# AvishaiBarnoy/membrane_solver

Measured on AMD Instinct MI355X. Metric: minimizer steps/sec (energy+grad+CG) on 2M-facet icosphere, higher is better.
Workload: dtype f64

## Files before the change

include/membrane_hip.h:

```cpp
#ifndef MEMBRANE_HIP_H
#define MEMBRANE_HIP_H

#include <stddef.h>
#include <stdint.h>

#ifdef __cplusplus
extern "C" {
#endif

#define MS_OK 0
#define MS_ERR_INVALID (-1)
#define MS_ERR_HIP (-2)
#define MS_ERR_TILE_CAPACITY (-3)
#define MS_ERR_STATE (-4)
#define MS_ERR_NOMEM (-5)

#define MS_MOD_SURFACE 1u
#define MS_MOD_BENDING 2u
#define MS_MOD_VOLUME_PENALTY 4u
#define MS_CON_VOLUME 8u
#define MS_TRACK_VOLUME 16u
#define MS_MOD_TILT 32u
#define MS_MOD_BENDING_TILT 64u
#define MS_MOD_TILT_SMOOTH 128u
// ... 266 lines not shown
int ms_rebind_state(ms_ctx *ctx, void *device_base, size_t bytes);

int ms_device_buffer(ms_ctx *ctx, int buffer, void **dev_ptr, size_t *bytes);
int ms_shard_info(ms_ctx *ctx, int64_t *nvp, int64_t *row0, int64_t *row1,
                  int64_t *rows_per_shard);
int ms_tile_stats(ms_ctx *ctx, int64_t *n_tiles, int64_t *facet_instances,
                  int64_t *max_halo, int64_t *lds_bytes_energy,
                  int64_t *lds_bytes_gradient);

#define MS_PROF_KINDS 13
int ms_profile_enable(ms_ctx *ctx, int on);
int ms_profile_read(ms_ctx *ctx, double total_ms[MS_PROF_KINDS],
                    int64_t launches[MS_PROF_KINDS]);

int ms_queue_stats(ms_ctx *ctx, int64_t stats[8]);
int ms_exec_stats(ms_ctx *ctx, int64_t stats[4]);
int ms_resident_stats(ms_ctx *ctx, int64_t stats[4]);

#define MS_PIN_STAGE_FIXED 0
#define MS_PIN_STAGE_PLANE_GROUP 1
#define MS_PIN_STAGE_CIRCLE_GROUP 2
#define MS_PIN_OP_PLANE 0
#define MS_PIN_OP_CIRCLE 1
#define MS_PIN_GRAD_PLANE 0
#define MS_PIN_GRAD_CIRCLE 1
#define MS_PIN_GRAD_RADIAL 2
#define MS_PIN_LANE_SKIP 0
#define MS_PIN_LANE_PROJECT 1
int ms_set_pins(ms_ctx *ctx, int n_params, const double *params, int n_stages, const int32_t *stage_kind,
                const int32_t *stage_param, const int32_t *stage_off, const int32_t *item_row,
// ... 36 lines not shown
```

membrane_solver_amd/_lib.py:

```python

from __future__ import annotations

import ctypes
import os
import subprocess

_PKG = os.path.dirname(os.path.abspath(__file__))
LIB_PATH = os.environ.get("MEMBRANE_HIP_LIB") or os.path.join(_PKG, "libmembrane_hip.so")
_CSRC = os.path.join(_PKG, "csrc")

MS_OK = 0
MS_ERR = {-1: "MS_ERR_INVALID", -2: "MS_ERR_HIP", -3: "MS_ERR_TILE_CAPACITY",
          -4: "MS_ERR_STATE", -5: "MS_ERR_NOMEM"}

MS_MOD_SURFACE = 1
MS_MOD_BENDING = 2
MS_MOD_VOLUME_PENALTY = 4
MS_CON_VOLUME = 8
MS_TRACK_VOLUME = 16
MS_MOD_TILT = 32
MS_MOD_BENDING_TILT = 64
MS_MOD_TILT_SMOOTH = 128
MS_MOD_TILT_IN, MS_MOD_TILT_OUT, MS_MOD_TILT_SMOOTH_IN, MS_MOD_TILT_SMOOTH_OUT = 256, 512, 1024, 2048
MS_MOD_BENDING_TILT_IN, MS_MOD_BENDING_TILT_OUT = 4096, 8192
# ... 158 lines not shown
    "ms_shard_exchange_count": (ctypes.c_int64, [_P]),
    "ms_shard_chain_stats": (ctypes.c_int, [_P, _I64]),
    "ms_shard_comm_ranks": (ctypes.c_int, [_P]),
    "ms_shard_peer_memory_kind": (ctypes.c_int, [_P]),
    "ms_state_bytes": (ctypes.c_size_t, [_P]),
    "ms_rebind_state": (ctypes.c_int, [_P, _P, ctypes.c_size_t]),
    "ms_fetch_scalars": (ctypes.c_int, [_P, _D]),
    "ms_store_scalars": (ctypes.c_int, [_P, _D]),
    "ms_device_buffer": (ctypes.c_int, [_P, ctypes.c_int, ctypes.POINTER(_P),
                                        ctypes.POINTER(ctypes.c_size_t)]),
    "ms_shard_info": (ctypes.c_int, [_P, _I64, _I64, _I64, _I64]),
    "ms_tile_stats": (ctypes.c_int, [_P, _I64, _I64, _I64, _I64, _I64]),
    "ms_profile_enable": (ctypes.c_int, [_P, ctypes.c_int]),
    "ms_profile_read": (ctypes.c_int, [_P, _D, _I64]),
    "ms_queue_stats": (ctypes.c_int, [_P, _I64]),
    "ms_exec_stats": (ctypes.c_int, [_P, _I64]),
    "ms_resident_stats": (ctypes.c_int, [_P, _I64]),
    "ms_set_pins": (ctypes.c_int, [_P, ctypes.c_int, _D, ctypes.c_int, _I32, _I32, _I32, _I32, _I32, ctypes.c_int,
                                   ctypes.c_int, _I32, _I32, _I32, ctypes.c_int, _I32, _I32, _I32]),
    "ms_enforce_pins": (ctypes.c_int, [_P]),
    "ms_pin_stats": (ctypes.c_int, [_P, _I64]),
    "ms_tsearch_stats": (ctypes.c_int, [_P, _I64]),
    "ms_exec_trace": (ctypes.c_int, [_P, ctypes.c_int, _D, ctypes.c_int, ctypes.POINTER(ctypes.c_int)]),
    "ms_shard_peer_export": (ctypes.c_int, [_P, _P]),
    "ms_shard_peer_open": (ctypes.c_int, [_P, _P]),
    "ms_shard_peer_local": (ctypes.c_int, [_P, ctypes.POINTER(_P), ctypes.POINTER(_P)]),
    "ms_shard_peer_set_pointers": (ctypes.c_int, [_P, ctypes.POINTER(_P), ctypes.POINTER(_P)]),
    "ms_shard_peer_set_barrier": (ctypes.c_int, [_P, _P, _P]),
    "ms_plan_tiling": (ctypes.c_int, [ctypes.c_int, ctypes.c_int, _D, _I32, ctypes.c_int, ctypes.c_int,
                                      _I64, _I32]),
# ... 88 lines not shown
```

membrane_solver_amd/csrc/ms_api_ctx.inc:

```
struct StageCtl {
  const uint32_t* cur_gate = nullptr;
  uint32_t cur_gate_want = 0;
  bool cur_gate_fold_only = false;
  bool cur_check_ran = false;
  uint32_t* cur_dec = nullptr;
  double cur_rhs[MS_MAX_TRIALS] = {0};
  const double* cur_rhs_dev = nullptr;
  uint32_t cur_extra_mask = 0;
  int cur_go_kind = 0;
  uint32_t* cur_go = nullptr;
  double cur_go_val[6] = {0};
  int cur_parity = 0;
  int pair_on = 0;
  bool pair_lean = false;
  double pair_alpha[MS_MAX_TRIALS] = {0};
  double* pair_scal2 = nullptr;
  bool multi_any_slot = false;
  bool defer_dir = false;
  bool energy_tilt_only = false;
  bool proj_at_x_in_normals = false;
};
struct CarryState {
  bool dir_implicit = false;
  bool pd_neg_pg = false;
  bool kc_pending = false;
  int kc_parity = 0;
  bool bt_valid = false;
  double* last_g = nullptr;
  bool cg_have_history = false;
  int cg_iter_count = 0;
  bool factors_valid = false;
  bool carry_valid = false;
  bool grad_valid = false;
  bool maxg2_valid = false;
};
struct ms_ctx {
  int device = 0;
  hipStream_t stream = nullptr;
// ... 70 lines not shown
    bool implicit = false;
    double alpha0 = 0, energy0 = 0, beta = 0, c1 = 0, tol2p = 0, lim = 0;
    RoundPlanT plan;
  } ahead;
  bool ahead_enable = true;
  int steps_left = 0;
  bool ahead_allowed = false;
  uint32_t dir_deferred_mask = 0;
  bool dir_pending[2] = {false, false};
  uint32_t dir_mask[2] = {0, 0};
  uint32_t* kc_gate[2] = {nullptr, nullptr};
  bool last_hist_descent = false;
  long q_ahead = 0, q_adopted = 0, q_dropped = 0;
  int kc_stepper = 0;
  bool kc_use_history = false;
  uint32_t* d_dec = nullptr;
  static constexpr int N_DEC = 16;
  unsigned long long* h_err = nullptr;
  unsigned long long* d_h_err = nullptr;
  long queue_mismatches = 0;
  long q_rounds = 0, q_multi = 0, q_wasted = 0, q_side_accepts = 0;
  int escalate_after = 3;
  bool pair_enable = true;
  bool escalate = true;
  int pair_force = 0;
  bool lbt_normals_current = false;
  bool tenergy_enable = true;
  bool tsearch_enable = true;
  bool tsearch_first_single = true;
  int64_t tsearch_launches = 0, tsearch_trials = 0;
// ... 158 lines not shown
```

membrane_solver_amd/csrc/ms_api_misc.inc:

```
size_t ms_state_bytes(const ms_ctx* c) {
  if (!c) return 0;
  return sizeof(double) * (8 * 3 * (size_t)c->til.nvp + 2 * (size_t)c->til.nvp);
}

int ms_rebind_state(ms_ctx* c, void* device_base, size_t bytes) {
  if (!c || !device_base) return fail(c, MS_ERR_INVALID, "ms_rebind_state: NULL argument");
  const size_t need = ms_state_bytes(c);
  if (bytes < need) return fail(c, MS_ERR_INVALID, "ms_rebind_state: buffer smaller than ms_state_bytes");
  HIPCHK(c, hipStreamSynchronize(S(c)));
  HIPCHK(c, hipMemcpy(device_base, c->state, need, hipMemcpyDeviceToDevice));
  double* nb = static_cast<double*>(device_base);
  for (int b = 0; b <= MS_BUF_FA; ++b) c->buf[b] = nb + (c->buf[b] - c->state);
  c->carry.last_g = nb + (c->carry.last_g - c->state);
  if (c->own_state) HIPCHK(c, hipFree(c->state));
  c->state = nb;
  c->own_state = false;
  return MS_OK;
}

int ms_fetch_scalars(ms_ctx* c, double* out) {
  if (!c || !out) return MS_ERR_INVALID;
  int rc = fetch(c);
  if (rc) return rc;
  memcpy(out, c->h_scal, sizeof(double) * MS_NSCAL);
// ... 48 lines not shown
                                                      (c->params.modules & MS_CON_VOLUME) != 0, !c->deterministic);
  return MS_OK;
}

int ms_queue_stats(ms_ctx* c, int64_t stats[8]) {
  if (!c || !stats) return MS_ERR_INVALID;
  for (int k = 0; k < 8; ++k) stats[k] = 0;
  stats[0] = c->q_rounds;
  stats[1] = c->q_multi;
  stats[2] = c->q_wasted;
  stats[3] = c->q_side_accepts;
  stats[4] = c->queue_mismatches;
  stats[5] = c->q_ahead;
  stats[6] = c->q_adopted;
  stats[7] = c->q_dropped;
  return MS_OK;
}

int ms_resident_stats(ms_ctx* c, int64_t stats[4]) {
  if (!c || !stats) return MS_ERR_INVALID;
  stats[0] = c->resident_ok;
  stats[1] = c->resident_launches;
  stats[2] = c->resident_steps;
  stats[3] = c->resident_bails;
  return MS_OK;
}

int ms_tsearch_stats(ms_ctx* c, int64_t stats[2]) {
  if (!c || !stats) return MS_ERR_INVALID;
  stats[0] = c->tsearch_launches;
// ... 320 lines not shown
```

membrane_solver_amd/csrc/ms_api_phases.inc:

```
namespace {

inline hipStream_t S(ms_ctx* c) {
  if (c->exec_on) (void)c->exec.flush();
  return c->stream;
}
int pin_grad_run(ms_ctx* c, bool volrow);
inline int exec_flush(ms_ctx* c) {
  if (!c->exec_on) return MS_OK;
  const hipError_t e = c->exec.flush();
  if (e == hipSuccess) return MS_OK;
  c->err = std::string("k_exec launch: ") + hipGetErrorString(e);
  return MS_ERR_HIP;
}

inline int zero_doubles(ms_ctx* c, double* p, size_t bytes) {
  if (c->exec_on) {
    ExecMemsetArgs a;
    a.p = p;
    a.n = (int64_t)(bytes / sizeof(double));
    const hipError_t e = c->exec.push(CK_MEMSET, 0, 0, 0, 1, 0, 0, &a, sizeof(a));
    if (e == hipSuccess) return MS_OK;
    c->err = std::string("k_exec record: ") + hipGetErrorString(e);
    return MS_ERR_HIP;
  }
// ... 672 lines not shown
    if (!used) return fail(c, MS_ERR_STATE, "tilt energy pass: planned but not launched");
  }
  if (reduce_now) {
    constexpr uint32_t core = (1u << MS_S_ESURF) | (1u << MS_S_VOL) | (1u << MS_S_EBEND) | (1u << MS_S_MINEDGE2) |
                              (1u << MS_S_GUARD);
    int rc = reduce_slots(c, tilt_only ? (energy_mask(modules) & ~core) : energy_mask(modules));
    if (rc) return rc;
  }
  if (bend && write_factors) c->carry.factors_valid = !use_dir;
  if (!lbt) c->factors_leaflet = 0;
  c->carry.bt_valid = (bt || lbt) && !use_dir;
  return MS_OK;
}

int phase_gradient(ms_ctx* c, uint32_t modules_in, double* g_out, bool accumulate, int dir_mode = 0,
                   bool reduce_now = true) {
  uint32_t modules = modules_in;
  if ((modules & (MS_MOD_BENDING | MS_MOD_BENDING_TILT | MS_LEAFLET_BT)) && !c->carry.factors_valid)
    return fail(c, MS_ERR_STATE, "gradient pass needs the bending factors of an energy pass at x");
  if (modules & MS_MOD_BENDING_TILT)
    modules = (modules & ~MS_MOD_BENDING_TILT) | MS_MOD_BENDING;
  int lbt_order[2] = {0, 0}, n_lbt = 0;
  if (modules & MS_LEAFLET_BT) {
    if (dir_mode) return fail(c, MS_ERR_STATE, "bending_tilt_in/out cannot use the fused direction pass");
    if (modules & MS_MOD_BENDING) return fail(c, MS_ERR_STATE, "bending together with bending_tilt_in/out is outside the device path");
    if (c->params.bending_grad_mode != MS_GRAD_ANALYTIC)
      return fail(c, MS_ERR_STATE, "bending_tilt_in/out: only bending_gradient_mode=analytic is on the device path");
    for (int l = 2; l >= 1; --l)
      if (modules & c->tf[l].mod_bt) lbt_order[n_lbt++] = l;
    if (n_lbt == 2 && c->factors_leaflet == lbt_order[1]) std::swap(lbt_order[0], lbt_order[1]);
    modules |= MS_MOD_BENDING;
// ... 5 lines not shown
  a.x = c->buf[MS_BUF_X];
  a.fK = c->buf[MS_BUF_FK];
  a.fA = c->buf[MS_BUF_FA];
  a.g = g_out;
  a.gC = (modules & MS_CON_VOLUME) ? c->buf[MS_BUF_GC] : nullptr;
  a.partials = c->d_partials;
  a.scal = c->d_scal;
  a.modules = modules;
  a.bending_grad_mode = c->params.bending_grad_mode;
  a.volume_stiffness = c->params.volume_stiffness;
  a.target_volume = c->params.target_volume;
  a.area_stiffness = c->area_stiffness;
  a.target_area = c->target_area;
  a.accumulate = accumulate ? 1 : 0;
  a.dir_mode = dir_mode;
  a.d = c->buf[MS_BUF_D];
  a.pg = c->buf[MS_BUF_PG];
  a.pd = c->buf[MS_BUF_PD];
  a.pd_neg_pg = (dir_mode == 2 && c->carry.pd_neg_pg) ? 1 : 0;
  a.gate = c->stage().cur_gate;
  a.gate_want = c->stage().cur_gate_want;
  a.atomic = c->deterministic ? 0 : 1;
  a.bt_vert = nullptr;
  a.tilts = nullptr;
  a.div_sign = 1.0;
  if (n_lbt == 0) {
    ProfScope ps(c, gradient_lean_instance(a) ? 9 : 1, a.gate, a.gate_want);
    HIPCHK(c, launch_gradient(a, c->cap, c->til.max_ent, c->stream));
  }
  for (int k = 0; k < n_lbt; ++k) {
    TiltField& f = c->tf[lbt_order[k]];
// ... 13 lines not shown
    if (k > 0) {
      al.modules = MS_MOD_BENDING;
      al.gC = nullptr;
      al.accumulate = 1;
    }
    {
      ProfScope ps(c, 1);
      HIPCHK(c, launch_gradient(al, c->cap, c->til.max_ent, c->stream));
    }
    int rc = bt_pass_f(c, f, 3, false, 0.0, f.tilts);
    if (rc) return rc;
  }
  if (dir_mode) {
    c->carry.last_g = g_out;
    c->carry.dir_implicit = false;
  }
  bool added_after = n_lbt > 0;
  for (int k = 0; k < 3 && g_out; ++k) {
    TiltField& f = c->tf[k];
    if (modules & f.mod_tilt) {
      int rc = tilt_pass_f(c, f, 1, false, 0.0);
      if (rc) return rc;
      added_after = true;
    }
    if (k > 0 && (modules & f.mod_dt)) {
      int rc = disk_target_pass(c, f, 1, false, 0.0, f.tilts, true, false);
      if (rc) return rc;
      added_after = true;
    }
  }
  if (added_after && g_out && (modules & MS_CON_VOLUME))
    HIPCHK(c, launch_row_dot(c->tile0, c->tile1, c->til.nv, c->til.own, g_out, c->buf[MS_BUF_GC], c->d_partials,
                             c->til.n_tiles, c->stream));
  if (reduce_now) return reduce_slots(c, dir_mode ? MASK_DIR : MASK_GRAD);
  return MS_OK;
}

int phase_direction(ms_ctx* c, int stepper, bool use_history, bool g_finalized = false) {
  const bool use_con = (c->params.modules & MS_CON_VOLUME) != 0 && c->pin_lane != MS_PIN_LANE_SKIP;
  const StageCtl& st = c->stage();
  c->carry.dir_implicit = false;
  {
  ProfScope ps(c, 2, st.cur_gate, st.cur_gate_want);
  HIPCHK(c, launch_direction(c->tile0, c->tile1, c->til.nv, c->til.own, c->d_vflags, c->buf[MS_BUF_G],
                             c->buf[MS_BUF_GC], c->buf[MS_BUF_D], c->buf[MS_BUF_PG],
                             c->buf[MS_BUF_PD], c->d_scal, use_con ? 1 : 0,
                             (stepper == MS_STEPPER_CG && use_history) ? 1 : 0, c->d_partials,
                             c->til.n_tiles, (g_finalized && !use_con) ? 0 : 1, c->stream, st.cur_gate,
                             st.cur_gate_want,
                             (stepper == MS_STEPPER_CG && use_history && c->carry.pd_neg_pg) ? 1 : 0,
                             (stepper == MS_STEPPER_CG && c->precond) ? 1 : 0));
  }
  c->carry.last_g = c->buf[MS_BUF_G];
  return reduce_slots(c, MASK_DIR);
}

void put_mailbox(ms_ctx* c, int sl, double v) {
  c->h_scal[sl] = v;
  unsigned long long bits;
  memcpy(&bits, &v, sizeof(double));
  __atomic_store_n(&c->h_seq[2 * sl], bits, __ATOMIC_RELAXED);
  __atomic_store_n(&c->h_seq[2 * sl + 1], bits ^ c->expected[sl], __ATOMIC_RELAXED);
}

const char* box_name(ms_ctx* c, const void* h_seq);
bool trace_queue();

int check_queue_error(ms_ctx* c) {
  if (!c->h_err) return MS_OK;
  const unsigned long long e = __atomic_load_n(c->h_err, __ATOMIC_ACQUIRE);
// ... 109 lines not shown
    if (c->params.modules & f.mod_bt) e[1] += c->h_scal[f.s_ebt];
    if (c->params.modules & f.mod_dt) e[3] += c->h_scal[f.s_edt];
  }
}

int queue_energy_and_gradient(ms_ctx* c, int stepper, bool use_history, bool skip_energy = false) {
  const uint32_t mods = c->params.modules;
  const bool constraint = (mods & (MS_CON_VOLUME | MS_TILT_SHAPE_MODS)) != 0 || (stepper == MS_STEPPER_CG && c->precond) ||
                          c->pin_lane == MS_PIN_LANE_PROJECT;
  const bool penalty = skip_energy || (mods & (MS_MOD_VOLUME_PENALTY | MS_MOD_AREA_PENALTY)) != 0;
  int rc = MS_OK;
  if (!skip_energy) rc = phase_energy(c, mods, false, 0.0, false, false, true, penalty);
  if (rc) return rc;
  if (!constraint) {
    const int dir_mode = (stepper == MS_STEPPER_CG && use_history) ? 2 : 1;
    rc = phase_gradient(c, mods, c->buf[MS_BUF_G], false, dir_mode, false);
    if (rc) return rc;
    return reduce_slots(c, (penalty ? 0u : energy_mask(mods)) | MASK_DIR);
  }
  rc = phase_gradient(c, mods, c->buf[MS_BUF_G], false, 0, false);
  if (rc) return rc;
  rc = pin_grad_run(c, (mods & MS_CON_VOLUME) != 0);
  if (rc) return rc;
  const uint32_t gmask = (mods & (MS_CON_VOLUME | MS_TILT_SHAPE_MODS)) ? MASK_GRAD : 0u;
  const uint32_t fmask = (penalty ? 0u : energy_mask(mods)) | gmask;
  if (fmask) rc = reduce_slots(c, fmask);
  if (rc) return rc;
  return phase_direction(c, stepper, use_history);
}

template <typename Tp>
// ... 45 lines not shown
```

membrane_solver_amd/csrc/ms_api_shard.inc:

```
int ms_phase_energy(ms_ctx* c, int use_direction, double alpha, int write_trial, int guard,
                    int write_bending_factors) {
  if (!c) return MS_ERR_INVALID;
  if ((c->params.modules & MS_ANY_TILT_MODS) && c->shard_count != 1)
    return fail(c, MS_ERR_STATE, "the tilt module is not sharded yet (single GPU only)");
  return phase_energy(c, c->params.modules, use_direction != 0, alpha, write_trial != 0, guard != 0,
                      write_bending_factors != 0);
}

int ms_phase_gradient(ms_ctx* c) {
  if (!c) return MS_ERR_INVALID;
  c->carry.grad_valid = false;
  return phase_gradient(c, c->params.modules, c->buf[MS_BUF_G], false);
}

int ms_phase_direction(ms_ctx* c, int stepper, int use_history) {
  if (!c) return MS_ERR_INVALID;
  c->precond = false;
  return phase_direction(c, stepper, use_history != 0);
}

int ms_phase_accept(ms_ctx* c, int keep_history) {
  if (!c) return MS_ERR_INVALID;
  std::swap(c->buf[MS_BUF_X], c->buf[MS_BUF_XT]);
  c->carry.factors_valid = false;
  c->carry.carry_valid = c->carry.grad_valid = c->carry.bt_valid = c->carry.maxg2_valid = false;
  c->sh_carry_valid = c->sh_grad_valid = false;
  c->sh_maxg2_valid = false;
  if (keep_history) {
    std::swap(c->buf[MS_BUF_G], c->buf[MS_BUF_PG]);
    std::swap(c->buf[MS_BUF_D], c->buf[MS_BUF_PD]);
    c->carry.pd_neg_pg = c->carry.dir_implicit;
    c->carry.last_g = c->buf[MS_BUF_PG];
    c->carry.cg_have_history = true;
    ++c->carry.cg_iter_count;
  }
  c->carry.dir_implicit = false;
  return MS_OK;
}

int ms_phase_commit_trial(ms_ctx* c, double alpha, int keep_history) {
  if (!c) return MS_ERR_INVALID;
  if (c->shard_count > 1) {
    const Tiling& t = c->til;
    const int64_t rows_per = (int64_t)t.tiles_per_shard * t.own;
    HIPCHK(c, launch_axpy_rows(c->shard_rank * rows_per, (c->shard_rank + 1) * rows_per, c->d_halo_rows,
                               c->n_halo_rows, c->d_vflags, c->buf[MS_BUF_X], trial_dir(c), trial_alpha(c, alpha),
                               c->stream));
    std::swap(c->buf[MS_BUF_X], c->buf[MS_BUF_XT]);
    return ms_phase_accept(c, keep_history);
  }
  const size_t n3 = 3 * (size_t)c->til.nvp;
  HIPCHK(c, hipMemcpyAsync(c->buf[MS_BUF_XT], c->buf[MS_BUF_X], n3 * sizeof(double),
                           hipMemcpyDeviceToDevice, S(c)));
  HIPCHK(c, launch_axpy_masked(c->til.nvp, c->d_vflags, c->buf[MS_BUF_XT], trial_dir(c), trial_alpha(c, alpha),
                               c->stream));
  return ms_phase_accept(c, keep_history);
// ... 967 lines not shown
```

membrane_solver_amd/csrc/ms_api_step.inc:

```
int ms_set_positions(ms_ctx* c, const double* positions) {
  if (!c || !positions) return fail(c, MS_ERR_INVALID, "ms_set_positions: NULL argument");
  c->carry.factors_valid = false;
  c->carry.carry_valid = c->carry.grad_valid = c->carry.bt_valid = c->carry.maxg2_valid = false;
  c->sh_carry_valid = c->sh_grad_valid = false;
  return ext_to_patch(c, positions, c->buf[MS_BUF_X], 3);
}

int ms_get_positions(ms_ctx* c, double* positions) {
  if (!c || !positions) return fail(c, MS_ERR_INVALID, "ms_get_positions: NULL argument");
  return patch_to_ext(c, c->buf[MS_BUF_X], positions, 3);
}

int ms_get_gradient(ms_ctx* c, double* grad) {
  if (!c || !grad) return fail(c, MS_ERR_INVALID, "ms_get_gradient: NULL argument");
  return patch_to_ext(c, c->carry.last_g, grad, 3);
}

int ms_get_vertex_buffer(ms_ctx* c, int buffer, double* out) {
  if (!c || !out || buffer < 0 || buffer > MS_BUF_FA)
    return fail(c, MS_ERR_INVALID, "ms_get_vertex_buffer: bad argument");
  if ((buffer == MS_BUF_D && c->carry.dir_implicit) || (buffer == MS_BUF_PD && c->carry.pd_neg_pg)) {
    const int src = buffer == MS_BUF_D ? MS_BUF_G : MS_BUF_PG;
    HIPCHK(c, launch_direction(c->tile0, c->tile1, c->til.nv, c->til.own, c->d_vflags, c->buf[src], c->buf[MS_BUF_GC],
                               c->buf[buffer], c->buf[MS_BUF_PG], c->buf[MS_BUF_PD], c->d_scal, 0, 0, c->d_partials,
                               c->til.n_tiles, 0, c->stream));
    if (buffer == MS_BUF_D) c->carry.dir_implicit = false; else c->carry.pd_neg_pg = false;
  }
  return patch_to_ext(c, c->buf[buffer], out, buffer == MS_BUF_FA ? 2 : 3);
}

int ms_energy_and_gradient(ms_ctx* c, double energies[4], double* grad) {
  if (!c || !energies) return fail(c, MS_ERR_INVALID, "ms_energy_and_gradient: NULL argument");
  if (c->shard_count != 1)
    return fail(c, MS_ERR_STATE, "ms_energy_and_gradient: sharded contexts use the phase API");
  int rc = queue_energy_and_gradient(c, MS_STEPPER_GD, false);
  if (rc) return rc;
// ... 29 lines not shown
  if (c->shard_count != 1) return fail(c, MS_ERR_STATE, "ms_energy: sharded contexts use the phase API");
  if (c->carry.carry_valid) {
    energies_from_mailbox(c, energies);
    return MS_OK;
  }
  int rc = phase_energy(c, c->params.modules, false, 0.0, false, false, false);
  if (rc) return rc;
  rc = fetch(c);
  if (rc) return rc;
  energies_from_mailbox(c, energies);
  return MS_OK;
}

int ms_reset_stepper(ms_ctx* c) {
  if (!c) return MS_ERR_INVALID;
  c->carry.cg_have_history = false;
  c->carry.cg_iter_count = 0;
  c->carry.pd_neg_pg = false;
  return MS_OK;
}

namespace {
int spec_prepare(ms_ctx* c) {
  if (c->d_dec) return MS_OK;
  auto make_box = [&](ms_ctx::Mailbox& m) -> int { return make_mailbox(c, m); };
  if (c->pair_enable) {
    const size_t nvp = (size_t)std::max<int64_t>(1, c->til.nvp);
    HIPCHK(c, hipMalloc(reinterpret_cast<void**>(&c->xt2), sizeof(double) * 3 * nvp));
    HIPCHK(c, hipMalloc(reinterpret_cast<void**>(&c->fK2), sizeof(double) * 3 * nvp));
    HIPCHK(c, hipMalloc(reinterpret_cast<void**>(&c->fA2), sizeof(double) * 2 * nvp));
    if (c->shard_count == 1 && !c->pair_lean_enable) {
      HIPCHK(c, hipMalloc(reinterpret_cast<void**>(&c->xt3), sizeof(double) * 3 * nvp));
      HIPCHK(c, hipMalloc(reinterpret_cast<void**>(&c->fK3), sizeof(double) * 3 * nvp));
// ... 137 lines not shown
    if (cg) {
      std::swap(c->buf[MS_BUF_G], c->buf[MS_BUF_PG]);
      std::swap(c->buf[MS_BUF_D], c->buf[MS_BUF_PD]);
      c->carry.pd_neg_pg = c->carry.dir_implicit;
    }
    c->carry.factors_valid = true;
    swap_mailbox(c, c->grad_mb[parity]);
    StageCtl st;
    st.cur_gate = dec_word(c, parity, n_st);
    st.cur_gate_want = DEC_ACCEPT_MAIN;
    st.cur_check_ran = true;
    st.defer_dir = c->ahead_allowed && sp->edge_fraction <= 0.0;
    c->dir_deferred_mask = 0;
    StageScope scope(c, st);
    rc = queue_energy_and_gradient(c, sp->stepper, next_hist, true);
    c->dir_pending[parity] = st.defer_dir && c->dir_deferred_mask != 0;
    c->dir_mask[parity] = c->dir_deferred_mask;
    c->kc_gate[parity] = dec_word(c, parity, n_st);
    swap_mailbox(c, c->grad_mb[parity]);
    if (cg) {
      std::swap(c->buf[MS_BUF_G], c->buf[MS_BUF_PG]);
      std::swap(c->buf[MS_BUF_D], c->buf[MS_BUF_PD]);
    }
    std::swap(c->buf[MS_BUF_X], c->buf[MS_BUF_XT]);
    c->carry = s_carry;
    if (rc) return rc;
  }
  return MS_OK;
}

// ... 16 lines not shown
  const int p = c->ahead.parity;
  forget(c->first_mb[p]);
  forget(c->grad_mb[p]);
  for (auto& m : c->spec[p]) forget(m);
  for (auto& sd : c->side) forget(sd.mb[p]);
  c->dir_pending[p] = false;
  c->ahead.valid = false;
  ++c->q_dropped;
  if (ran >= 1) c->carry.factors_valid = false;
  if (ran >= 2) {
    c->carry.carry_valid = c->carry.grad_valid = c->carry.maxg2_valid = false;
    c->carry.kc_pending = false;
    c->carry.cg_have_history = false;
    c->carry.cg_iter_count = 0;
    c->carry.pd_neg_pg = false;
  }
}

int queue_ahead(ms_ctx* c, const ms_stepper_params* sp, const ms_step_result* out, double tol, bool carry_mode,
                bool cg, int restart) {
  if (!c->carry.kc_pending || c->ahead.valid) return MS_OK;
  const int src = c->carry.kc_parity;
  if (!c->dir_pending[src]) return MS_OK;
  const int kind = c->kc_use_history ? (c->last_hist_descent ? 3 : 1) : 2;
  const double alpha0 = out->next_step;
  const double me2 = c->h_scal[MS_S_MINEDGE2];
  if (c->steps_left < (kind == 1 ? 2 : 1) || !(alpha0 >= 1e-8) || sp->edge_fraction > 0.0)
    return flush_dir_fold(c, src);
  double a_hi, r_lo;
  const ms_ctx::LsHist& lh = c->ls[kind == 3 ? 1 : 0];
  ls_bounds(lh, a_hi, r_lo);
  const int max_iter = sp->max_iter > 0 ? sp->max_iter : 10;
  ms_ctx::Ahead& ah = c->ahead;
  plan_round(c, sp, alpha0, max_iter, 0, a_hi, r_lo, lh.n >= 2, lh.pred_trials, 0, ah.plan, true);
  if (ah.plan.n0 + ah.plan.n_st > MS_MAX_TRIALS) return flush_dir_fold(c, src);
  ah.kind = kind;
  ah.stepper = sp->stepper;
  ah.implicit = kind == 1;
  ah.alpha0 = alpha0;
// ... 4 lines not shown
  ah.tol2p = tol * tol * (1.0 + 1e-9);
  ah.lim = (c->til.nf > 0 && me2 > 0.0) ? (0.09 * me2 / (1.0 + 1e-9)) / (alpha0 * alpha0) : INFINITY;
  ah.src = src;
  ah.go = false;
  ah.go_known = false;
  ah.go_kind = kind == 1 ? 1 : 2;
  const CarryState s_carry = c->carry;
  if (kind == 1) {
    c->carry.cg_have_history = false;
    c->carry.cg_iter_count = 0;
    c->carry.pd_neg_pg = false;
    c->carry.dir_implicit = true;
  } else {
    c->carry.dir_implicit = false;
  }
  const int parity = c->next_parity;
  c->next_parity ^= 1;
  ah.parity = parity;
  int rc = queue_round(c, sp, ah.plan, parity, 0.0, 0.0, true, src, carry_mode, cg, restart);
  c->carry = s_carry;
  if (rc) return rc;
  ah.valid = true;
  ++c->q_ahead;
  return MS_OK;
}
}

int ms_step(ms_ctx* c, const ms_stepper_params* sp, double step_size, double tol,
            ms_step_result* out) {
  if (!c || !sp || !out) return fail(c, MS_ERR_INVALID, "ms_step: NULL argument");
// ... 11 lines not shown
  }
  const bool carried_x = carry_mode && c->carry.carry_valid;
  const bool carried = carried_x &&
                       (c->carry.factors_valid || !(c->params.modules & (MS_MOD_BENDING | MS_MOD_BENDING_TILT)));
  const bool volrow = (c->params.modules & MS_CON_VOLUME) != 0;
  const bool precond = cg && sp->precondition != 0;
  c->precond = precond;
  int rc;
  bool restart_sd = false;
  const bool tilt_shape = (c->params.modules & MS_TILT_SHAPE_MODS) != 0;
  if (carried_x && c->carry.grad_valid && !tilt_shape && c->til.T <= 256 &&
      (!volrow || (!use_history && c->carry.maxg2_valid && !precond))) {
    restart_sd = !use_history && c->carry.maxg2_valid && !precond;
    if (restart_sd) {
      c->carry.dir_implicit = true;
      c->carry.last_g = c->buf[MS_BUF_G];
      c->h_scal[MS_S_GDOTD] = -c->h_scal[MS_S_GNORM2];
      c->h_scal[MS_S_MAXD2] = c->h_scal[MS_S_MAXG2];
      rc = MS_OK;
    } else {
      rc = phase_direction(c, sp->stepper, use_history, true);
    }
  } else if (c->carry.kc_pending && carried_x && !(c->params.modules & MS_TILT_SHAPE_MODS) && c->kc_stepper == sp->stepper &&
             c->kc_use_history == use_history && !precond) {
    c->carry.kc_pending = false;
    double vals[MS_NSCAL];
    if (c->ahead.valid && !c->ahead.go_known && c->ahead.src == c->carry.kc_parity) {
      ms_ctx::Ahead& ah = c->ahead;
      uint32_t code = DEC_NONE;
      rc = wait_mailbox(c, c->first_mb[ah.parity].h_seq, c->first_mb[ah.parity].expected, vals, &code);
// ... 8 lines not shown
          if (rc) return rc;
        }
        ah.go = go;
      }
      if (!ah.go) drop_ahead(c, 1);
    } else {
      rc = flush_dir_fold(c, c->carry.kc_parity);
      if (rc) return rc;
      rc = wait_mailbox(c, c->grad_mb[c->carry.kc_parity].h_seq, c->grad_mb[c->carry.kc_parity].expected, vals, nullptr);
      if (rc) return rc;
    }
    for (int sl = 0; sl < MS_NSCAL; ++sl)
      if (MASK_DIR & (1u << sl)) put_mailbox(c, sl, vals[sl]);
    c->carry.last_g = c->buf[MS_BUF_G];
    c->carry.dir_implicit = false;
    c->carry.maxg2_valid = true;
  } else {
    c->carry.kc_pending = false;
    rc = queue_energy_and_gradient(c, sp->stepper, use_history, carried);
    c->carry.maxg2_valid = true;
  }
  if (rc) return rc;
  if (!restart_sd) {
    rc = fetch(c);
    if (rc) return rc;
  }
  c->carry.carry_valid = carry_mode;
  c->carry.grad_valid = carry_mode && !tilt_shape;
  double e[4];
  energies_from_mailbox(c, e);
  const double E_eval = e[0] + e[1] + e[2] + e[3];
  const double grad_norm = std::sqrt(c->h_scal[MS_S_GNORM2]);
  const double g_dot_d = c->h_scal[MS_S_GDOTD];
  const double max_dir = std::sqrt(c->h_scal[MS_S_MAXD2]);
  out->energy_eval = E_eval;
  out->grad_norm = grad_norm;
  out->g_dot_d = g_dot_d;
  out->volume = c->h_scal[MS_S_VOL];
  out->next_step = step_size;
  out->energy = E_eval;
  if (use_history) c->last_hist_descent = g_dot_d < 0.0;
// ... 17 lines not shown
    {
      StageScope scope(c, st);
      rc = phase_energy(c, c->params.modules, false, 0.0, false, false, false);
    }
    if (rc) return rc;
    rc = fetch(c);
    if (rc) return rc;
    energies_from_mailbox(c, e);
    energy0 = e[0] + e[1] + e[2] + e[3];
    min_edge = std::sqrt(c->h_scal[MS_S_MINEDGE2]);
  }
  if (c->til.nf == 0) min_edge = 0.0;
  out->energy = energy0;
  const double safe_step_limit = min_edge > 0.0 ? 0.3 * min_edge : INFINITY;
  if (g_dot_d >= 0.0) return MS_OK;
  double alpha = step_size;
  if (sp->edge_fraction > 0.0 && min_edge > 0.0 && max_dir > 0.0)
    alpha = std::min(alpha, sp->edge_fraction * min_edge / max_dir);
  const double alpha_max = sp->alpha_max_factor * step_size;
  const int max_iter = sp->max_iter > 0 ? sp->max_iter : 10;
  bool kc_queued = false;
  double min_rejected = INFINITY;
  double a_hi, r_lo;
  ms_ctx::LsHist& lh = c->ls[use_history ? 1 : 0];
  ls_bounds(lh, a_hi, r_lo);
  const bool ls_warm = lh.n >= 2;
  auto accept = [&](double alpha_acc, double E_t) {
    std::swap(c->buf[MS_BUF_X], c->buf[MS_BUF_XT]);
    c->carry.factors_valid = carry_mode;
    c->carry.carry_valid = carry_mode;
// ... 355 lines not shown
  c->resident_steps += ro->steps;
  if (trace_steps())
    fprintf(stderr, "[mss] resident launch: asked %d steps from step size %.3e -> took %d, reason %d, %d barriers\n", n,
            step_size, ro->steps, ro->reason, (int)res[7]);
  if (trace_steps() && ro->steps > 0)
    fprintf(stderr, "[mss]   per step (us, workgroup 0): gradient %.2f | barrier %.2f | lambda+rows+direction %.2f | trial energies "
                    "%.2f | barrier %.2f | fold %.2f\n", res[8] / ro->steps, res[9] / ro->steps, res[10] / ro->steps,
            res[11] / ro->steps, res[12] / ro->steps, res[13] / ro->steps);
  if (ro->steps > 0) {
    c->h_res_log.resize((size_t)8 * ro->steps);
    HIPCHK(c, hipMemcpy(c->h_res_log.data(), c->d_res_log, sizeof(double) * 8 * (size_t)ro->steps, hipMemcpyDeviceToHost));
  }
  c->carry.carry_valid = c->carry.grad_valid = c->carry.factors_valid = c->carry.maxg2_valid = c->carry.bt_valid = false;
  c->carry.kc_pending = false;
  c->carry.dir_implicit = false;
  if (ro->reason == RES_TIMEOUT) return fail(c, MS_ERR_STATE, "resident step kernel: a grid barrier timed out");
  return MS_OK;
}
}

int ms_minimize(ms_ctx* c, const ms_minimize_params* mp, int n_steps, ms_minimize_result* out,
                double* step_log) {
  if (!c || !mp || !out) return fail(c, MS_ERR_INVALID, "ms_minimize: NULL argument");
  memset(out, 0, sizeof(*out));
  double step_size = mp->step_size;
  int zero_steps = 0;
  out->step_success = 1;
  out->step_size = step_size;
  const bool resident = resident_eligible(c, mp);
  int resident_cooldown = 0;
// ... 159 lines not shown
```

membrane_solver_amd/csrc/ms_kernels.hip:

```cpp
#include <hip/hip_runtime.h>
#include <atomic>
#include <cstddef>
#include <cstdio>
#include <cstdlib>
#include <cstring>
#include <ctime>
#include <mutex>
#include <type_traits>

#include "ms_internal.h"

#ifndef MS_RSQRT_NORM
#define MS_RSQRT_NORM 1
#endif

namespace ms {

struct V3 {
  double x, y, z;
};
__device__ __forceinline__ V3 mk(double x, double y, double z) { return V3{x, y, z}; }
__device__ __forceinline__ V3 operator-(V3 a, V3 b) { return mk(a.x - b.x, a.y - b.y, a.z - b.z); }
__device__ __forceinline__ V3 operator+(V3 a, V3 b) { return mk(a.x + b.x, a.y + b.y, a.z + b.z); }
__device__ __forceinline__ V3 operator-(V3 a) { return mk(-a.x, -a.y, -a.z); }
// ... 1020 lines not shown
        okp = a.m.kappa[v_own];
        ot0 = a.tilts[g];
        ot1 = a.tilts[g + 1];
        ot2 = a.tilts[g + 2];
      }
    }
    CsrStage cs;
    if (!ATOMIC) csr_issue(cs, a.m, t, T, tid);
    if (ATOMIC) {
      for (int j = tid; j < NACC * T; j += T) stg[j] = 0.0;
    }
    double hx0 = 0, hx1 = 0, hx2 = 0, hk0 = 0, hk1 = 0, hk2 = 0, hae = 0, hav = 0;
    uint8_t hfl = 0;
    if (has_h) {
      const size_t g = 3 * (size_t)hv;
      hfl = a.m.vflags[hv];
      hx0 = a.x[g];
      hx1 = a.x[g + 1];
      hx2 = a.x[g + 2];
      if (BEND) {
        hk0 = a.fK[g];
        hk1 = a.fK[g + 1];
        hk2 = a.fK[g + 2];
        hae = LEAF ? a.bt_vert[4 * (size_t)hv] : a.fA[2 * (size_t)hv];
        hav = a.fA[2 * (size_t)hv + 1];
      }
      if (LEAF) {
        hkp = a.m.kappa[hv];
        ht0 = a.tilts[g];
        ht1 = a.tilts[g + 1];
        ht2 = a.tilts[g + 2];
// ... 13 lines not shown
      }
      if (LEAF) {
        kp[tid] = okp;
        tl[tid] = ot0;
        tl[cap + tid] = ot1;
        tl[2 * cap + tid] = ot2;
      }
    }
    if (!ATOMIC) {
      csr_commit(cs, a.m, t, T, tid, vent);
      cur = cs.vo0;
      end = cs.vo1;
    }
    if (has_h) {
      const int s = t.n_owned + tid;
      lfl[s] = hfl;
      lds_put3(px, s, hx0, hx1, hx2);
      if (BEND) {
        lds_put3(fk, s, hk0, hk1, hk2);
        if (LEAN) {
          fa[s] = hae + hav;
        } else {
          fa[2 * s] = hae;
          fa[2 * s + 1] = hav;
        }
      }
      if (LEAF) {
        kp[s] = hkp;
        tl[s] = ht0;
        tl[cap + s] = ht1;
        tl[2 * cap + s] = ht2;
      }
    }
    for (int h = tid + T; h < t.nh; h += T) {
      const int v = a.m.halo_ids[t.h0 + h];
      const int s = t.n_owned + h;
      lfl[s] = a.m.vflags[v];
#pragma unroll
      for (int c = 0; c < 3; ++c) {
        px[3 * s + c] = a.x[3 * (size_t)v + c];
        if (BEND) fk[3 * s + c] = a.fK[3 * (size_t)v + c];
        if (LEAF) tl[c * cap + s] = a.tilts[3 * (size_t)v + c];
      }
      if (BEND && LEAN) {
        fa[s] = a.fA[2 * (size_t)v] + a.fA[2 * (size_t)v + 1];
      } else if (BEND) {
        fa[2 * s] = LEAF ? a.bt_vert[4 * (size_t)v] : a.fA[2 * (size_t)v];
        fa[2 * s + 1] = a.fA[2 * (size_t)v + 1];
      }
      if (LEAF) kp[s] = a.m.kappa[v];
    }
  }
// ... 320 lines not shown
      V3 gi = fixed ? mk(0, 0, 0) : mk(gx, gy, gz);
      V3 di = -gi;
      if (a.dir_mode == 2) {
        const V3 pgv = h_pg;
        const double beta = dot_pinned(gi, gi - pgv) / (dot_pinned(pgv, pgv) + 1.0e-20);
        if (!(beta < 0.0)) {
          const V3 q = h_pd;
          di = mk(fma(beta, q.x, -gi.x), fma(beta, q.y, -gi.y), fma(beta, q.z, -gi.z));
        }
      }
      if (fixed) di = mk(0, 0, 0);
      if (!MS_ABL_NOSTORE) {
        a.g[o] = gi.x;
        a.g[o + 1] = gi.y;
        a.g[o + 2] = gi.z;
        a.d[o] = di.x;
        a.d[o + 1] = di.y;
        a.d[o + 2] = di.z;
      }
      gn2 = dot_pinned(gi, gi);
      gdd = dot_pinned(gi, di);
      md2 = fixed ? 0.0 : dot_pinned(di, di);
      mg2 = gn2;
    } else if (a.g) {
      if (a.accumulate) {
        gx += a.g[o];
        gy += a.g[o + 1];
        gz += a.g[o + 2];
      }
      a.g[o] = gx;
      a.g[o + 1] = gy;
      a.g[o + 2] = gz;
    }
// ... 1886 lines not shown
```

membrane_solver_amd/device.py:

```python

from __future__ import annotations

import ctypes
from dataclasses import dataclass

import numpy as np

from . import _lib as L


def _f64(a, shape=None, name="array"):
    a = np.ascontiguousarray(a, dtype=np.float64)
    if shape is not None and a.shape != tuple(shape):
        raise ValueError(f"{name} must have shape {tuple(shape)}, got {a.shape}")
    return a


def _pd(a):
    return None if a is None else a.ctypes.data_as(L._D)


def _pu8(a):
    return None if a is None else a.ctypes.data_as(L._U8)

# ... 461 lines not shown
    def profile_read(self):
        ms = np.zeros(13)
        n = np.zeros(13, dtype=np.int64)
        self._chk(L.lib().ms_profile_read(self._h, _pd(ms), n.ctypes.data_as(L._I64)), "ms_profile_read")
        names = ("energy", "gradient", "direction", "reduce", "tilt", "bending_tilt", "tilt_vec", "energy_pair", "energy_triple",
                 "gradient_lean", "energy_multi", "tilt_smoothness", "tilt_search")
        return {k: (float(ms[i]), int(n[i])) for i, k in enumerate(names)}

    def queue_stats(self):
        v = np.zeros(8, dtype=np.int64)
        self._chk(L.lib().ms_queue_stats(self._h, v.ctypes.data_as(L._I64)), "ms_queue_stats")
        return {"rounds": int(v[0]), "multi_launches": int(v[1]), "wasted_evaluations": int(v[2]),
                "side_accepts": int(v[3]), "mismatches": int(v[4]), "ahead": int(v[5]), "adopted": int(v[6]),
                "dropped": int(v[7])}

    def exec_stats(self):
        v = np.zeros(4, dtype=np.int64)
        self._chk(L.lib().ms_exec_stats(self._h, v.ctypes.data_as(L._I64)), "ms_exec_stats")
        return {"active": bool(v[0]), "packs": int(v[1]), "launches_recorded": int(v[2]), "wanted": bool(v[3] & 1),
                "relax_programs": int((v[3] >> 8) & 0xffffff), "relax_fused": int(v[3] >> 32)}

    def set_pins(self, tables):
        if tables is None:
            self._chk(L.lib().ms_set_pins(self._h, 0, None, 0, None, None, None, None, None, 0, 0, None, None, None,
                                          0, None, None, None), "ms_set_pins")
            return

        def i32(v):
            return np.ascontiguousarray(np.asarray(v, dtype=np.int32).reshape(-1)) if len(v) else np.zeros(1, np.int32)

# ... 54 lines not shown
```

Before: 18190.

## Defer CG direction writes in fused gradient pass until needed

In the fused CG gradient pass, the search direction is no longer stored to the D buffer when conditions allow (single shard, no preconditioner, no volume constraint or tilt-shape modules). The direction stays implicit and is built by a separate direction kernel only when a later consumer needs it: trial energy, accept, commit, buffer readback, stepper reset or line search. This removes a 3-double-per-vertex store from the gradient kernel on steps where the direction is never read, at the cost of state-tracking complexity and an extra launch on steps where it is. The lean kernel path also stops loading and storing halo vertex flags in LDS.

After: 18590 (median of 6 runs). 2.2% higher.

```diff
diff --git a/include/membrane_hip.h b/include/membrane_hip.h
--- a/include/membrane_hip.h
+++ b/include/membrane_hip.h
@@ -304,6 +304,7 @@
                     int64_t launches[MS_PROF_KINDS]);
 
 int ms_queue_stats(ms_ctx *ctx, int64_t stats[8]);
+int ms_direction_stats(ms_ctx *ctx, int64_t *skipped, int64_t *materialized);
 int ms_exec_stats(ms_ctx *ctx, int64_t stats[4]);
 int ms_resident_stats(ms_ctx *ctx, int64_t stats[4]);
 
diff --git a/membrane_solver_amd/_lib.py b/membrane_solver_amd/_lib.py
--- a/membrane_solver_amd/_lib.py
+++ b/membrane_solver_amd/_lib.py
@@ -196,6 +196,7 @@
     "ms_profile_enable": (ctypes.c_int, [_P, ctypes.c_int]),
     "ms_profile_read": (ctypes.c_int, [_P, _D, _I64]),
     "ms_queue_stats": (ctypes.c_int, [_P, _I64]),
+    "ms_direction_stats": (ctypes.c_int, [_P, _I64, _I64]),
     "ms_exec_stats": (ctypes.c_int, [_P, _I64]),
     "ms_resident_stats": (ctypes.c_int, [_P, _I64]),
     "ms_set_pins": (ctypes.c_int, [_P, ctypes.c_int, _D, ctypes.c_int, _I32, _I32, _I32, _I32, _I32, ctypes.c_int,
diff --git a/membrane_solver_amd/csrc/ms_api_ctx.inc b/membrane_solver_amd/csrc/ms_api_ctx.inc
--- a/membrane_solver_amd/csrc/ms_api_ctx.inc
+++ b/membrane_solver_amd/csrc/ms_api_ctx.inc
@@ -22,6 +22,7 @@
 };
 struct CarryState {
   bool dir_implicit = false;
+  bool dir_unwritten = false;
   bool pd_neg_pg = false;
   bool kc_pending = false;
   int kc_parity = 0;
@@ -122,6 +123,8 @@
   long q_ahead = 0, q_adopted = 0, q_dropped = 0;
   int kc_stepper = 0;
   bool kc_use_history = false;
+  bool kc_dir_unwritten[2] = {false, false};
+  long dir_skipped = 0, dir_materialized = 0;
   uint32_t* d_dec = nullptr;
   static constexpr int N_DEC = 16;
   unsigned long long* h_err = nullptr;
diff --git a/membrane_solver_amd/csrc/ms_api_misc.inc b/membrane_solver_amd/csrc/ms_api_misc.inc
--- a/membrane_solver_amd/csrc/ms_api_misc.inc
+++ b/membrane_solver_amd/csrc/ms_api_misc.inc
@@ -86,6 +86,13 @@
   stats[5] = c->q_ahead;
   stats[6] = c->q_adopted;
   stats[7] = c->q_dropped;
+  return MS_OK;
+}
+
+int ms_direction_stats(ms_ctx* c, int64_t* skipped, int64_t* materialized) {
+  if (!c || !skipped || !materialized) return MS_ERR_INVALID;
+  *skipped = c->dir_skipped;
+  *materialized = c->dir_materialized;
   return MS_OK;
 }
 
diff --git a/membrane_solver_amd/csrc/ms_api_phases.inc b/membrane_solver_amd/csrc/ms_api_phases.inc
--- a/membrane_solver_amd/csrc/ms_api_phases.inc
+++ b/membrane_solver_amd/csrc/ms_api_phases.inc
@@ -710,7 +710,7 @@
 }
 
 int phase_gradient(ms_ctx* c, uint32_t modules_in, double* g_out, bool accumulate, int dir_mode = 0,
-                   bool reduce_now = true) {
+                   bool reduce_now = true, bool may_skip_d = false) {
   uint32_t modules = modules_in;
   if ((modules & (MS_MOD_BENDING | MS_MOD_BENDING_TILT | MS_LEAFLET_BT)) && !c->carry.factors_valid)
     return fail(c, MS_ERR_STATE, "gradient pass needs the bending factors of an energy pass at x");
@@ -746,7 +746,9 @@
   a.target_area = c->target_area;
   a.accumulate = accumulate ? 1 : 0;
   a.dir_mode = dir_mode;
-  a.d = c->buf[MS_BUF_D];
+  const bool skip_d = may_skip_d && dir_mode == 2 && c->shard_count == 1 && !c->last_hist_descent && !c->precond &&
+                      !(modules & (MS_CON_VOLUME | MS_TILT_SHAPE_MODS)) && c->pin_lane != MS_PIN_LANE_PROJECT;
+  a.d = skip_d ? nullptr : c->buf[MS_BUF_D];
   a.pg = c->buf[MS_BUF_PG];
   a.pd = c->buf[MS_BUF_PD];
   a.pd_neg_pg = (dir_mode == 2 && c->carry.pd_neg_pg) ? 1 : 0;
@@ -790,6 +792,7 @@
   if (dir_mode) {
     c->carry.last_g = g_out;
     c->carry.dir_implicit = false;
+    c->carry.dir_unwritten = skip_d;
   }
   bool added_after = n_lbt > 0;
   for (int k = 0; k < 3 && g_out; ++k) {
@@ -816,6 +819,7 @@
   const bool use_con = (c->params.modules & MS_CON_VOLUME) != 0 && c->pin_lane != MS_PIN_LANE_SKIP;
   const StageCtl& st = c->stage();
   c->carry.dir_implicit = false;
+  c->carry.dir_unwritten = false;
   {
   ProfScope ps(c, 2, st.cur_gate, st.cur_gate_want);
   HIPCHK(c, launch_direction(c->tile0, c->tile1, c->til.nv, c->til.own, c->d_vflags, c->buf[MS_BUF_G],
@@ -830,6 +834,18 @@
   c->carry.last_g = c->buf[MS_BUF_G];
   return reduce_slots(c, MASK_DIR);
 }
+
+int materialize_direction(ms_ctx* c, bool& flag) {
+  if (!flag) return MS_OK;
+  HIPCHK(c, launch_direction(c->tile0, c->tile1, c->til.nv, c->til.own, c->d_vflags, c->buf[MS_BUF_G], c->buf[MS_BUF_GC],
+                             c->buf[MS_BUF_D], c->buf[MS_BUF_PG], c->buf[MS_BUF_PD], c->d_scal, 0, 1,
+                             c->d_partials, c->til.n_tiles, 0, c->stream, nullptr, 0,
+                             c->carry.pd_neg_pg ? 1 : 0, 0));
+  flag = false;
+  ++c->dir_materialized;
+  return MS_OK;
+}
+int materialize_direction(ms_ctx* c) { return materialize_direction(c, c->carry.dir_unwritten); }
 
 void put_mailbox(ms_ctx* c, int sl, double v) {
   c->h_scal[sl] = v;
@@ -969,7 +985,7 @@
   if (rc) return rc;
   if (!constraint) {
     const int dir_mode = (stepper == MS_STEPPER_CG && use_history) ? 2 : 1;
-    rc = phase_gradient(c, mods, c->buf[MS_BUF_G], false, dir_mode, false);
+    rc = phase_gradient(c, mods, c->buf[MS_BUF_G], false, dir_mode, false, true);
     if (rc) return rc;
     return reduce_slots(c, (penalty ? 0u : energy_mask(mods)) | MASK_DIR);
   }
diff --git a/membrane_solver_amd/csrc/ms_api_shard.inc b/membrane_solver_amd/csrc/ms_api_shard.inc
--- a/membrane_solver_amd/csrc/ms_api_shard.inc
+++ b/membrane_solver_amd/csrc/ms_api_shard.inc
@@ -3,6 +3,8 @@
   if (!c) return MS_ERR_INVALID;
   if ((c->params.modules & MS_ANY_TILT_MODS) && c->shard_count != 1)
     return fail(c, MS_ERR_STATE, "the tilt module is not sharded yet (single GPU only)");
+  if (use_direction)
+    if (int rc = materialize_direction(c)) return rc;
   return phase_energy(c, c->params.modules, use_direction != 0, alpha, write_trial != 0, guard != 0,
                       write_bending_factors != 0);
 }
@@ -21,6 +23,7 @@
 
 int ms_phase_accept(ms_ctx* c, int keep_history) {
   if (!c) return MS_ERR_INVALID;
+  if (int rc = materialize_direction(c)) return rc;
   std::swap(c->buf[MS_BUF_X], c->buf[MS_BUF_XT]);
   c->carry.factors_valid = false;
   c->carry.carry_valid = c->carry.grad_valid = c->carry.bt_valid = c->carry.maxg2_valid = false;
@@ -40,6 +43,7 @@
 
 int ms_phase_commit_trial(ms_ctx* c, double alpha, int keep_history) {
   if (!c) return MS_ERR_INVALID;
+  if (int rc = materialize_direction(c)) return rc;
   if (c->shard_count > 1) {
     const Tiling& t = c->til;
     const int64_t rows_per = (int64_t)t.tiles_per_shard * t.own;
diff --git a/membrane_solver_amd/csrc/ms_api_step.inc b/membrane_solver_amd/csrc/ms_api_step.inc
--- a/membrane_solver_amd/csrc/ms_api_step.inc
+++ b/membrane_solver_amd/csrc/ms_api_step.inc
@@ -19,7 +19,11 @@
 int ms_get_vertex_buffer(ms_ctx* c, int buffer, double* out) {
   if (!c || !out || buffer < 0 || buffer > MS_BUF_FA)
     return fail(c, MS_ERR_INVALID, "ms_get_vertex_buffer: bad argument");
-  if ((buffer == MS_BUF_D && c->carry.dir_implicit) || (buffer == MS_BUF_PD && c->carry.pd_neg_pg)) {
+  if (buffer == MS_BUF_D && c->carry.kc_pending) {
+    if (int rc = materialize_direction(c, c->kc_dir_unwritten[c->carry.kc_parity])) return rc;
+  } else if (buffer == MS_BUF_D && c->carry.dir_unwritten) {
+    if (int rc = materialize_direction(c)) return rc;
+  } else if ((buffer == MS_BUF_D && c->carry.dir_implicit) || (buffer == MS_BUF_PD && c->carry.pd_neg_pg)) {
     const int src = buffer == MS_BUF_D ? MS_BUF_G : MS_BUF_PG;
     HIPCHK(c, launch_direction(c->tile0, c->tile1, c->til.nv, c->til.own, c->d_vflags, c->buf[src], c->buf[MS_BUF_GC],
                                c->buf[buffer], c->buf[MS_BUF_PG], c->buf[MS_BUF_PD], c->d_scal, 0, 0, c->d_partials,
@@ -79,9 +83,12 @@
 
 int ms_reset_stepper(ms_ctx* c) {
   if (!c) return MS_ERR_INVALID;
+  if (c->carry.kc_pending)
+    if (int rc = materialize_direction(c, c->kc_dir_unwritten[c->carry.kc_parity])) return rc;
   c->carry.cg_have_history = false;
   c->carry.cg_iter_count = 0;
   c->carry.pd_neg_pg = false;
+  c->carry.dir_unwritten = false;
   return MS_OK;
 }
 
@@ -249,6 +256,7 @@
     c->dir_deferred_mask = 0;
     StageScope scope(c, st);
     rc = queue_energy_and_gradient(c, sp->stepper, next_hist, true);
+    c->kc_dir_unwritten[parity] = c->carry.dir_unwritten;
     c->dir_pending[parity] = st.defer_dir && c->dir_deferred_mask != 0;
     c->dir_mask[parity] = c->dir_deferred_mask;
     c->kc_gate[parity] = dec_word(c, parity, n_st);
@@ -295,6 +303,7 @@
     c->carry.cg_have_history = false;
     c->carry.cg_iter_count = 0;
     c->carry.pd_neg_pg = false;
+    c->carry.dir_unwritten = false;
   }
 }
 
@@ -304,6 +313,7 @@
   const int src = c->carry.kc_parity;
   if (!c->dir_pending[src]) return MS_OK;
   const int kind = c->kc_use_history ? (c->last_hist_descent ? 3 : 1) : 2;
+  if (kind == 3 && c->kc_dir_unwritten[src]) return flush_dir_fold(c, src);
   const double alpha0 = out->next_step;
   const double me2 = c->h_scal[MS_S_MINEDGE2];
   if (c->steps_left < (kind == 1 ? 2 : 1) || !(alpha0 >= 1e-8) || sp->edge_fraction > 0.0)
@@ -338,6 +348,7 @@
   } else {
     c->carry.dir_implicit = false;
   }
+  c->carry.dir_unwritten = false;
   const int parity = c->next_parity;
   c->next_parity ^= 1;
   ah.parity = parity;
@@ -379,6 +390,7 @@
     restart_sd = !use_history && c->carry.maxg2_valid && !precond;
     if (restart_sd) {
       c->carry.dir_implicit = true;
+      c->carry.dir_unwritten = false;
       c->carry.last_g = c->buf[MS_BUF_G];
       c->h_scal[MS_S_GDOTD] = -c->h_scal[MS_S_GNORM2];
       c->h_scal[MS_S_MAXD2] = c->h_scal[MS_S_MAXG2];
@@ -417,6 +429,7 @@
       if (MASK_DIR & (1u << sl)) put_mailbox(c, sl, vals[sl]);
     c->carry.last_g = c->buf[MS_BUF_G];
     c->carry.dir_implicit = false;
+    c->carry.dir_unwritten = c->kc_dir_unwritten[c->carry.kc_parity];
     c->carry.maxg2_valid = true;
   } else {
     c->carry.kc_pending = false;
@@ -428,6 +441,7 @@
     rc = fetch(c);
     if (rc) return rc;
   }
+  if (c->carry.dir_unwritten) ++c->dir_skipped;
   c->carry.carry_valid = carry_mode;
   c->carry.grad_valid = carry_mode && !tilt_shape;
   double e[4];
@@ -475,6 +489,8 @@
   out->energy = energy0;
   const double safe_step_limit = min_edge > 0.0 ? 0.3 * min_edge : INFINITY;
   if (g_dot_d >= 0.0) return MS_OK;
+  rc = materialize_direction(c);
+  if (rc) return rc;
   double alpha = step_size;
   if (sp->edge_fraction > 0.0 && min_edge > 0.0 && max_dir > 0.0)
     alpha = std::min(alpha, sp->edge_fraction * min_edge / max_dir);
@@ -860,6 +876,7 @@
   c->carry.carry_valid = c->carry.grad_valid = c->carry.factors_valid = c->carry.maxg2_valid = c->carry.bt_valid = false;
   c->carry.kc_pending = false;
   c->carry.dir_implicit = false;
+  c->carry.dir_unwritten = false;
   if (ro->reason == RES_TIMEOUT) return fail(c, MS_ERR_STATE, "resident step kernel: a grid barrier timed out");
   return MS_OK;
 }
diff --git a/membrane_solver_amd/csrc/ms_kernels.hip b/membrane_solver_amd/csrc/ms_kernels.hip
--- a/membrane_solver_amd/csrc/ms_kernels.hip
+++ b/membrane_solver_amd/csrc/ms_kernels.hip
@@ -1058,7 +1058,7 @@
     uint8_t hfl = 0;
     if (has_h) {
       const size_t g = 3 * (size_t)hv;
-      hfl = a.m.vflags[hv];
+      if (!LEAN) hfl = a.m.vflags[hv];
       hx0 = a.x[g];
       hx1 = a.x[g + 1];
       hx2 = a.x[g + 2];
@@ -1102,7 +1102,7 @@
     }
     if (has_h) {
       const int s = t.n_owned + tid;
-      lfl[s] = hfl;
+      if (!LEAN) lfl[s] = hfl;
       lds_put3(px, s, hx0, hx1, hx2);
       if (BEND) {
         lds_put3(fk, s, hk0, hk1, hk2);
@@ -1123,7 +1123,7 @@
     for (int h = tid + T; h < t.nh; h += T) {
       const int v = a.m.halo_ids[t.h0 + h];
       const int s = t.n_owned + h;
-      lfl[s] = a.m.vflags[v];
+      if (!LEAN) lfl[s] = a.m.vflags[v];
 #pragma unroll
       for (int c = 0; c < 3; ++c) {
         px[3 * s + c] = a.x[3 * (size_t)v + c];
@@ -1474,9 +1474,11 @@
         a.g[o] = gi.x;
         a.g[o + 1] = gi.y;
         a.g[o + 2] = gi.z;
-        a.d[o] = di.x;
-        a.d[o + 1] = di.y;
-        a.d[o + 2] = di.z;
+        if (a.d != nullptr) {
+          a.d[o] = di.x;
+          a.d[o + 1] = di.y;
+          a.d[o + 2] = di.z;
+        }
       }
       gn2 = dot_pinned(gi, gi);
       gdd = dot_pinned(gi, di);
diff --git a/membrane_solver_amd/device.py b/membrane_solver_amd/device.py
--- a/membrane_solver_amd/device.py
+++ b/membrane_solver_amd/device.py
@@ -499,6 +499,12 @@
                 "side_accepts": int(v[3]), "mismatches": int(v[4]), "ahead": int(v[5]), "adopted": int(v[6]),
                 "dropped": int(v[7])}
 
+    def direction_stats(self):
+        v = np.zeros(2, dtype=np.int64)
+        self._chk(L.lib().ms_direction_stats(self._h, v[0:1].ctypes.data_as(L._I64), v[1:2].ctypes.data_as(L._I64)),
+                  "ms_direction_stats")
+        return {"skipped": int(v[0]), "materialized": int(v[1])}
+
     def exec_stats(self):
         v = np.zeros(4, dtype=np.int64)
         self._chk(L.lib().ms_exec_stats(self._h, v.ctypes.data_as(L._I64)), "ms_exec_stats")
```
